# NVlabs/intrinsic3d

Measured on NVIDIA H100. Metric: gauss_newton_iterations_per_sec, higher is better.
Workload: dtype f32

## Files before the change

### intrinsic3d_b200/csrc/i3d_engine.cu

```cuda
#include <cuda_runtime.h>
#include <dlfcn.h>

#include <algorithm>
#include <chrono>
#include <climits>
#include <cmath>
#include <cstdarg>
#include <cstdio>
#include <cstdlib>
#include <cstring>
#include <string>
#include <vector>

#include "../../include/i3d_c_api.h"
#include "i3d_kernels.cuh"
#include "i3d_lighting.cuh"
#include "i3d_recolor.cuh"
#include "i3d_gridops.cuh"
#include "i3d_host.h"
#include "i3d_frames.h"
#include "i3d_fusion.h"
#include "i3d_mesh.h"
#include "i3d_render.h"
#include "i3d_texture.h"
// ... 69 lines not shown
    Dev<int32_t> up_xyz, up_vals; Dev<uint8_t> up_rgb; Dev<unsigned long long> up_keys; Dev<int> up_dup; Dev<double> up_sh;
    uint64_t hash_cap = 0;
    Dev<int32_t> sp_x, sp_y, sp_z; Dev<double> sp_sdf0, sp_sdf, sp_alb; Dev<float> sp_w; Dev<uchar4> sp_rgb;
    Dev<int32_t> act, scan_counts, scan_total;
    int n_active = 0, K = 0, stride = 0;
    Dev<float> Rt;
    Dev<FramePose> pose_ctx, pose_ctx_c;
    Dev<int32_t> obs_frame, row_frame;
    Dev<float> obs_w;
    Dev<float4> Jt;
    Dev<float2> Jtail;
    Dev<double> row_res, row_wraw;
    Dev<float> ea_w;
    Dev<double> lap;
    Dev<float> cam_acc;
    Dev<double> minv, type_w;
    Dev<int> fail_flag;
    Dev<float> v_bg, v_cg, v_s, v_jtj, v_b, v_x, v_r, v_z, v_p, v_ps, v_qg, v_tr, v_delta;
    Dev<double> v_bgd, v_cgd, v_qgd, cam_accd;
    Dev<CgCtl> ctl;
    Dev<double> red_partials, red_out;
    Dev<unsigned int> red_counters;
    size_t max_blocks = 0;
    bool keep_raw = false;
    Dev<float> dbg_v;
    I3DParams last_params{};
    bool have_iter = false;
    Timing timing;
    int64_t launches = 0;
    int64_t host_syncs = 0;
    Dev<IterDev> iter_dev;
    int last_cg_iterations = 4, prev_cg_iterations = 4;
    bool pcg_fused = true;
    int64_t step_n = -1;
    unsigned step_grid = 0; int step_K = 0; size_t step_smem = 0;
    Dev<uint8_t> color;
    bool have_color = false;
    Dev<unsigned long long> recolor_counts;
    Dev<int32_t> sv_table, sv_index, sv_nbr;
    Dev<int> sv_scalars, sv_deg;
    Dev<double> sv_acc, sv_work;
    Dev<I3DLightingInfo> sv_info;
    Dev<uint8_t> sh_has;
    int sv_S = 0;
    double* sv_x = nullptr;
    SubvolGrid sv_grid{};
    FusionState fusion;
    ScoreScratch scores;
    RgbdStore rgbd;
    SensorStore sensor;
    MeshState mesh;
    TextureState tex;
    DistanceState dist;
    RenderState render;
    TrackScratch track;
    int64_t shard_begin = 0, shard_end = -1;
    int rank = 0, world = 1;
    NcclApi::Comm comm = nullptr;
    bool shard_ready = false;
    Dev<uint8_t> held;
    Dev<uint8_t> held_mask;
    Dev<int32_t> slist;
    int64_t n_shared = 0;
    int64_t hv0 = 0, hv1 = 0;
    int64_t loc_begin = 0, loc_end = 0;
    Dev<double> xbuf;
// ... 264 lines not shown
        return;
    }
    NK(g_nccl.AllReduce(dev, dev, static_cast<size_t>(count), NCCL_FLOAT64, NCCL_SUM, e->comm, e->stream));
    if (kind >= 0) pdl_launch(e, k_epilogue, 1, 32, 0, e->ctl.p, dev, kind, respect_done);
}

void exchange(I3DEngine* e, float* v0, float* v1, float* extra_f, int n_extra_f, double* extra_d, int n_extra_d, int respect_done, int epilogue_kind = -1)
{
    if (e->world <= 1) return;
    const ShareView shv = e->share_view();
    const size_t nv = v1 ? 2 : 1;
    const size_t total = nv * static_cast<size_t>(e->n_shared) + n_extra_f + n_extra_d;
    const size_t threads = static_cast<size_t>(e->n_shared) + n_extra_f + n_extra_d;
    if (e->p2p_ready && total <= e->mbox_cap)
    {
        const unsigned int seq = ++e->xseq;
        double* buf = reinterpret_cast<double*>(e->mbox.p + I3DEngine::kMboxFlagBytes) + static_cast<size_t>(seq & 1u) * e->mbox_cap;
        pdl_launch(e, k_pack, blocks_for(threads), kThreads, 0, shv, v0, v1, extra_f, n_extra_f, extra_d, n_extra_d, buf, e->ctl.p, respect_done);
        pdl_launch(e, k_xchg_pull, blocks_for(threads), kThreads, 0, e->p2p_view(), seq, shv, v0, v1, extra_f, n_extra_f, extra_d, n_extra_d, e->ctl.p, respect_done, epilogue_kind);
        return;
    }
    e->xbuf.ensure(2 * static_cast<size_t>(e->n_shared) + CamAccLayout{e->F}.size() + 64);
    pdl_launch(e, k_pack, blocks_for(threads), kThreads, 0, shv, v0, v1, extra_f, n_extra_f, extra_d, n_extra_d, e->xbuf.p, e->ctl.p, respect_done);
    NK(g_nccl.AllReduce(e->xbuf.p, e->xbuf.p, total, NCCL_FLOAT64, NCCL_SUM, e->comm, e->stream));
    pdl_launch(e, k_unpack, blocks_for(threads), kThreads, 0, shv, v0, v1, extra_f, n_extra_f, extra_d, n_extra_d, e->xbuf.p, e->ctl.p, respect_done);
    if (epilogue_kind >= 0) pdl_launch(e, k_epilogue, 1, 32, 0, e->ctl.p, extra_d, epilogue_kind, respect_done);
}

size_t apply_smem_bytes(int F, int K)
{
    return static_cast<size_t>((6 * F + 9 + 15) & ~15) * sizeof(double) + static_cast<size_t>(14 + 6 * K) * kThreads * sizeof(float);
}

size_t accum_smem_bytes(int F, int K)
{
    return static_cast<size_t>((CamAccLayout{F}.size() + 15) & ~15) * sizeof(double) + static_cast<size_t>(K) * 8 * kThreads * sizeof(float);
}

int check_frame_limit(I3DEngine* e, int F, int K)
{
    int optin = 0;
    CK(cudaDeviceGetAttribute(&optin, cudaDevAttrMaxSharedMemoryPerBlockOptin, e->device));
    cudaFuncAttributes fa_acc{}, fa_app{};
    CK(cudaFuncGetAttributes(&fa_acc, k_eg_accum));
    CK(cudaFuncGetAttributes(&fa_app, k_eg_apply));
    const size_t lim = static_cast<size_t>(optin);
    auto fits = [&](int f) { return fa_acc.sharedSizeBytes + accum_smem_bytes(f, K) <= lim && fa_app.sharedSizeBytes + apply_smem_bytes(f, K) <= lim; };
    if (fits(F)) return 0;
    int fmax = 0;
    while (fits(fmax + 1)) ++fmax;
    return fail(e, "i3d_gn_iteration: %d frames at K = %d observations need %zu bytes of shared memory per block in k_eg_accum (device limit %d): "
                   "at most %d frames at K = %d", F, K, fa_acc.sharedSizeBytes + accum_smem_bytes(F, K), optin, fmax, K);
}

void launch_eg_apply(I3DEngine* e, const GridView& g, const RegView& rv, const EgRows& rows, const SolveVecs& sv)
{
    if (rows.n_active == 0) return;
    Timer kt(e->timing, e->stream, "k_eg_apply");
    pdl_launch(e, k_eg_apply, blocks_for(rows.n_active), kThreads, apply_smem_bytes(e->F, rows.K), g, rows, rv, sv, sv.ps, e->ctl.p, e->site(SITE_EG_APPLY));
}

void launch_operator(I3DEngine* e, const GridView& g, const RegView& rv, const EgRows& rows, const SolveVecs& sv, const Shard& sh, const float* vin,
                     float dmin, float dmax, int is_cg_iteration)
{
    launch_eg_apply(e, g, rv, rows, sv);
    {
        Timer kt(e->timing, e->stream, "k_op_partial", 1);
        pdl_launch(e, k_op_partial, blocks_for(static_cast<size_t>((e->held_count() + 3) / 4)), kThreads, 0,
            g, rv, sv, sh, e->held_count(), vin, sv.ps, e->type_w.p, dmin, dmax, e->ctl.p, e->site(SITE_OP_POST), e->site(SITE_EG_APPLY).out, is_cg_iteration);
    }
    if (e->world > 1)
    {
        Timer kt(e->timing, e->stream, "exchange", 1);
        exchange(e, sv.qg, nullptr, sv.qg + 2 * e->n, 6 * e->F + 9, e->site(SITE_OP_POST).out, 1, 1, is_cg_iteration ? EPI_OPERATOR_CG : -1);
    }
}

bool plan_cg_step(I3DEngine* e)
{
    if (e->step_n == e->n) return e->step_grid > 0;
    e->step_n = e->n; e->step_grid = 0;
    int sms = 0, optin = 0;
    CK(cudaDeviceGetAttribute(&sms, cudaDevAttrMultiProcessorCount, e->device));
    CK(cudaDeviceGetAttribute(&optin, cudaDevAttrMaxSharedMemoryPerBlockOptin, e->device));
    cudaFuncAttributes fa0{}, fa1{};
// ... 100 lines not shown
        const size_t smem = 12 * static_cast<size_t>(F) * sizeof(float);
        auto kern = (K <= 5) ? k_select_obs<5> : k_select_obs<I3D_MAX_OBS>;
        if (smem > 48 * 1024) CK(cudaFuncSetAttribute(kern, cudaFuncAttributeMaxDynamicSharedMemorySize, static_cast<int>(smem)));
        Timer kt(e->timing, e->stream, "k_select_obs");
        static const bool want_stats = std::getenv("I3D_CULL_STATS") != nullptr;
        e->cull_stats.ensure(2);
        if (want_stats) CK(cudaMemsetAsync(e->cull_stats.p, 0, 2 * sizeof(unsigned long long), st));
        const CullView cull = cull_view(e, want_stats ? e->cull_stats.p : nullptr);
        pdl_launch(e, kern, blocks_for(static_cast<size_t>(n_active)), kThreads, smem, g, e->frame_view(), e->Rt.p, sc, cull, n_active, stride, e->act.p, K,
                                                                                e->obs_frame.p, e->obs_w.p);
        if (want_stats)
        {
            unsigned long long hs[2] = {0, 0};
            CK(cudaMemcpyAsync(hs, e->cull_stats.p, sizeof(hs), cudaMemcpyDeviceToHost, st));
            CK(cudaStreamSynchronize(st));
            fprintf(stderr, "[i3d] frame culling: %llu of %llu (warp, frame) pairs visited (%.1f %%)\n", hs[0], hs[1], hs[1] ? 100.0 * hs[0] / hs[1] : 0.0);
        }
    }
    t_sel.stop();

    Timer t_build(e->timing, e->stream, "build");
    e->Jt.ensure(EgRows::kTiles * S + 1); e->Jtail.ensure(S + 1);
    e->row_frame.ensure(S + 1); e->row_res.ensure(S + 1); e->row_wraw.ensure(S + 1);
    e->ea_w.ensure(3 * static_cast<size_t>(n)); e->lap.ensure(n);
    CK(cudaFuncSetAttribute(k_eg_apply, cudaFuncAttributeMaxDynamicSharedMemorySize, static_cast<int>(apply_smem_bytes(F, K))));
    const EgRows rows = eg_rows(e);
    CamView cv{e->cam, e->pose_ctx.p, F};
    if (n_active > 0)
    {
        {
            Timer kt(e->timing, e->stream, "k_eg_build");
            launch_eg_rows<ROWS_BUILD>(e, g, cv, rows, e->obs_frame.p, e->obs_w.p);
        }
        const size_t smem = accum_smem_bytes(F, K);
        if (smem > 48 * 1024) CK(cudaFuncSetAttribute(k_eg_accum, cudaFuncAttributeMaxDynamicSharedMemorySize, static_cast<int>(smem)));
        {
            Timer kt(e->timing, e->stream, "k_eg_accum", 1);
            pdl_launch(e, k_eg_accum, blocks_for(static_cast<size_t>(n_active)), kThreads, smem, g, rows, F, e->v_bgd.p, e->v_cgd.p, e->cam_accd.p, e->site(SITE_BUILD));
        }
        pdl_launch(e, k_acc_to_float, blocks_for(std::max(U, static_cast<size_t>(lay.size()))), kThreads, 0, static_cast<int64_t>(U), lay.size(),
                   e->v_bgd.p, e->v_cgd.p, e->cam_accd.p, e->v_bg.p, e->v_cg.p, e->cam_acc.p);
    }
    const RegView rv = reg_view(e, P);
    pdl_launch(e, k_reg_build, blocks_for(static_cast<size_t>((sh.loc_end - sh.loc_begin + 3) / 4)), kThreads, 0, g, rv, sh, e->site(SITE_REG));
    {
        const double na = static_cast<double>(n_active);
        CK(cudaMemcpyAsync(e->site(SITE_BUILD).out + 3, &na, sizeof(double), cudaMemcpyHostToDevice, st));
    }
    if (multi) exchange(e, e->v_bg.p, e->v_cg.p, e->cam_acc.p, lay.size(), e->red_out.p, 2 * kSiteVals, 0);
    pdl_launch(e, k_type_weights, 1, 32, 0, e->iter_dev.p, e->site(SITE_BUILD).out, e->site(SITE_REG).out, P, n, e->type_w.p);
    if (S > 0) pdl_launch(e, k_row_weights, blocks_for(S), kThreads, 0, rows, e->type_w.p);
    SolveVecs sv = solve_vecs(e);
    pdl_launch(e, k_finish_problem, blocks_for(static_cast<size_t>((hc + 3) / 4)), kThreads, 0, g, rv, sv, sh, hc, e->type_w.p, e->cam_acc.p, P.fix_poses, P.fix_intrinsics,
                                                                              P.fix_distortion, P.gradient_tolerance, e->site(SITE_FINISH), e->cam);
    allreduce_scalars(e, e->site(SITE_FINISH).out, 3, -1, 0);
    pdl_launch(e, k_iter_finish, 1, 32, 0, e->iter_dev.p, e->site(SITE_FINISH).out, P);
    t_build.stop();
    e->have_iter = true;
    if (P.build_only)
    {
        IterDev hb{};
        CK(cudaMemcpyAsync(&hb, e->iter_dev.p, sizeof(hb), cudaMemcpyDeviceToHost, st));
        sync();
        CK(cudaGetLastError());
        info = hb.info;
        t_total.stop();
        return 0;
    }

    Timer t_solve(e->timing, e->stream, "solve");
    const float dmin = static_cast<float>(P.min_lm_diagonal), dmax = static_cast<float>(std::min(P.max_lm_diagonal, 3.0e38));
// ... 234 lines not shown

extern "C" {

int i3d_abi_version(void) { return I3D_ABI_VERSION; }
uint64_t i3d_sizeof_params(void) { return sizeof(I3DParams); }
uint64_t i3d_sizeof_iter_info(void) { return sizeof(I3DIterInfo); }

void i3d_default_params(I3DParams* p)
{
    std::memset(p, 0, sizeof(*p));
    p->lambda[0] = 0.2; p->lambda[1] = 80.0; p->lambda[2] = 120.0; p->lambda[3] = 0.1;
    p->use_er = p->use_es = p->use_ea = 1;
    p->occlusion_distance = 0.02f; p->num_observations = 5; p->lm_steps = 50;
    p->initial_trust_region_radius = 1e4; p->max_trust_region_radius = 1e16; p->min_trust_region_radius = 1e-32;
    p->min_relative_decrease = 1e-3; p->min_lm_diagonal = 1e-6; p->max_lm_diagonal = 1e32; p->eta = 0.1;
    p->function_tolerance = 1e-6; p->gradient_tolerance = 1e-10; p->parameter_tolerance = 1e-8;
    p->max_linear_solver_iterations = 500; p->min_linear_solver_iterations = 0; p->residual_reset_period = 10;
    p->max_consecutive_invalid_steps = 5;
}

int i3d_engine_create(int device, I3DEngine** out)
{
    *out = nullptr;
    int count = 0;
    cudaError_t err = cudaGetDeviceCount(&count);
    if (err != cudaSuccess || count <= 0) return fail(nullptr, "i3d_engine_create: no CUDA device available (%s); this engine has no CPU fallback", cudaGetErrorString(err));
    if (device < 0 || device >= count) return fail(nullptr, "i3d_engine_create: device %d out of range (%d devices)", device, count);
    cudaDeviceProp prop;
    if (cudaGetDeviceProperties(&prop, device) != cudaSuccess) return fail(nullptr, "i3d_engine_create: cannot query device %d", device);
    if (prop.major != 9 || prop.minor != 0) return fail(nullptr, "i3d_engine_create: device %d is sm_%d%d; this library is built for sm_90a (H100) only", device, prop.major, prop.minor);
    I3DEngine* e = new I3DEngine();
    e->device = device;
    { const char* v = std::getenv("I3D_PCG_FUSED"); e->pcg_fused = !(v && v[0] == '0'); }
    const int rc = guarded(e, [&]() {
        CK(cudaStreamCreateWithFlags(&e->stream, cudaStreamNonBlocking));
        e->timing.pool.resize(4096);
        for (auto& ev : e->timing.pool) CK(cudaEventCreate(&ev));
        return 0;
    });
    if (rc != 0) { g_create_error = e->error; delete e; return rc; }
    *out = e;
    return 0;
}

void i3d_engine_destroy(I3DEngine* e)
{
    if (!e) return;
    cudaSetDevice(e->device);
    cudaStreamSynchronize(e->stream);
    for (size_t r = 0; r < e->peer_base.size(); ++r)
        if (static_cast<int>(r) != e->rank && e->peer_base[r]) cudaIpcCloseMemHandle(e->peer_base[r]);
    if (e->comm && g_nccl.CommDestroy) g_nccl.CommDestroy(e->comm);
    for (auto& ev : e->timing.pool) cudaEventDestroy(ev);
    if (e->mesh.ev_ready) for (auto& ev : e->mesh.ev) cudaEventDestroy(ev);
    if (e->tex.ev_ready) for (auto& ev : e->tex.ev) cudaEventDestroy(ev);
    cudaStreamDestroy(e->stream);
    delete e;
}

const char* i3d_last_error(const I3DEngine* e) { return e ? e->error.c_str() : g_create_error.c_str(); }

int i3d_upload_grid(I3DEngine* e, int64_t n, const int32_t* xyz, const double* sdf0, const double* sdf_refined, const double* albedo,
                    const float* weight, const uint8_t* rgb, float voxel_size)
{
    if (!e) return 1;
    if (n <= 0 || n > (1ll << 30)) return fail(e, "i3d_upload_grid: bad voxel count %lld", static_cast<long long>(n));
// ... 1529 lines not shown
```

### intrinsic3d_b200/csrc/i3d_kernels.cuh

```cuda
#pragma once
#include <cuda_runtime.h>
#include <cooperative_groups.h>
#include <stdint.h>
#include <limits.h>
#include "i3d_math.cuh"
#include "i3d_grid.cuh"
#include "i3d_observe.cuh"
#include "../../include/i3d_types.h"

namespace i3d
{

enum : uint8_t { FL_VALID = 1, FL_ACTIVE = 2, FL_RING = 4, FL_FREE_SDF = 8, FL_FREE_ALB = 16, FL_ES_JAC = 32, FL_ROW = 64  };

struct Shard
{
    int64_t own_begin, own_end;
    int64_t hv0, hv1;
    int cam_owner;
    int defer;
    int64_t loc_begin, loc_end;
    __device__ __forceinline__ bool owns_voxel(int64_t v) const { return v >= own_begin && v < own_end; }
    __device__ __forceinline__ bool owns_unknown(int64_t j, int64_t n) const
    {
// ... 422 lines not shown
struct EgRows
{
    int n_active, K;
    int stride;
    const int32_t* act;
    float4* Jt;
    float2* Jtail;
    int32_t* row_frame;
    double* row_res;
    double* row_wraw;
    static constexpr int kTiles = 7;
    __host__ __device__ size_t slots() const { return static_cast<size_t>(K) * stride; }
    __device__ __forceinline__ void store_row(size_t slot, const float row[29]) const
    {
        const size_t S = slots();
#pragma unroll
        for (int c = 0; c < kTiles; ++c) Jt[c * S + slot] = make_float4(row[4 * c], row[4 * c + 1], row[4 * c + 2], row[4 * c + 3]);
        Jtail[slot].x = row[28];
    }
    template <bool STREAM>
    __device__ __forceinline__ float load_row(size_t slot, float jr[29]) const
    {
        const size_t S = slots();
#pragma unroll
        for (int c = 0; c < kTiles; ++c)
        {
            const float4 t = STREAM ? __ldcs(Jt + c * S + slot) : Jt[c * S + slot];
            jr[4 * c] = t.x; jr[4 * c + 1] = t.y; jr[4 * c + 2] = t.z; jr[4 * c + 3] = t.w;
        }
        const float2 t = STREAM ? __ldcs(Jtail + slot) : Jtail[slot];
        jr[28] = t.x;
        return t.y;
    }
};

__device__ __forceinline__ void make_cam_params(const CamView& cv, double pyr_scale, int W, int H, CamParams<double>* c)
{
    const double* intr = cv.cam + 6 * cv.F;
    const double* dist = intr + 4;
    c->fx = intr[0] * pyr_scale; c->fy = intr[1] * pyr_scale; c->cx = intr[2] * pyr_scale; c->cy = intr[3] * pyr_scale;
    c->k1 = dist[0]; c->k2 = dist[1]; c->k3 = dist[2]; c->p1 = dist[3]; c->p2 = dist[4];
    c->pyr_scale = pyr_scale; c->w = W; c->h = H;
}

__device__ __forceinline__ bool gather_stencil(const GridView& g, const double* __restrict__ sdf, const double* __restrict__ alb, int64_t v,
                                               int32_t idx[14], double s10[10], double a4[4])
{
    const int64_t n = g.n;
    const int32_t xp = g.nbr[NB_XP * n + v], yp = g.nbr[NB_YP * n + v], zp = g.nbr[NB_ZP * n + v];
    const int32_t x2 = g.nbr[NB_X2 * n + v], y2 = g.nbr[NB_Y2 * n + v], z2 = g.nbr[NB_Z2 * n + v];
    const int32_t xy = g.nbr[NB_XY * n + v], xz = g.nbr[NB_XZ * n + v], yz = g.nbr[NB_YZ * n + v];
    idx[0] = static_cast<int32_t>(v); idx[1] = yp; idx[2] = y2; idx[3] = yz; idx[4] = zp; idx[5] = z2; idx[6] = xp; idx[7] = xy; idx[8] = xz; idx[9] = x2;
    idx[10] = static_cast<int32_t>(v); idx[11] = xp; idx[12] = yp; idx[13] = zp;
    bool ok = true;
#pragma unroll
    for (int k = 0; k < 10; ++k) ok = ok && (idx[k] >= 0);
    if (!ok) return false;
#pragma unroll
    for (int k = 0; k < 10; ++k) s10[k] = sdf[idx[k]];
#pragma unroll
    for (int k = 0; k < 4; ++k) a4[k] = alb[idx[10 + k]];
    return true;
}

__device__ __forceinline__ double sdf_to_weight(double sdf, double truncation)
{
    const double a = fmin(fabs(sdf), truncation) / truncation;
    return fmin(fmax(1.0 - a, 0.01), 1.0);
}

struct CamAccLayout
{
    int F;
    __host__ __device__ int pose_stride() const { return 33; }
    __host__ __device__ int tail() const { return 33 * F; }
    __host__ __device__ int size() const { return 33 * F + 43; }
};

enum { ROWS_BUILD = 0, ROWS_COST = 1 };
constexpr int kRowThreads = 128;

__device__ __forceinline__ uint32_t smem_u32(const void* p) { return static_cast<uint32_t>(__cvta_generic_to_shared(p)); }
__device__ __forceinline__ void mbar_init(uint64_t* bar, uint32_t count)
{
    asm volatile("mbarrier.init.shared::cta.b64 [%0], %1;" ::"r"(smem_u32(bar)), "r"(count) : "memory");
    asm volatile("fence.mbarrier_init.release.cluster;" ::: "memory");
}
__device__ __forceinline__ void mbar_expect_tx(uint64_t* bar, uint32_t bytes)
{
    asm volatile("mbarrier.arrive.expect_tx.shared::cta.b64 _, [%0], %1;" ::"r"(smem_u32(bar)), "r"(bytes) : "memory");
}
__device__ __forceinline__ void bulk_copy_g2s(void* dst_smem, const void* src_gmem, uint32_t bytes , uint64_t* bar)
{
    asm volatile("cp.async.bulk.shared::cluster.global.mbarrier::complete_tx::bytes [%0], [%1], %2, [%3];"
                 ::"r"(smem_u32(dst_smem)), "l"(src_gmem), "r"(bytes), "r"(smem_u32(bar)) : "memory");
}
__device__ __forceinline__ void mbar_wait(uint64_t* bar, uint32_t parity)
{
    uint32_t done = 0;
    while (!done)
        asm volatile("{\n\t.reg .pred P1;\n\tmbarrier.try_wait.parity.shared::cta.b64 P1, [%1], %2;\n\tselp.b32 %0, 1, 0, P1;\n\t}"
                     : "=r"(done) : "r"(smem_u32(bar)), "r"(parity) : "memory");
}

static_assert(kVoxelGeomWords == 15, "VoxelGeom size changed: update the pose-table staging boundary and its test");
__host__ __device__ inline size_t rows_pose_bytes(int F) { return (static_cast<size_t>(F) * sizeof(FramePose) + 127) & ~static_cast<size_t>(127); }
__host__ __device__ inline size_t rows_smem_bytes(int mode, int threads, bool stage, int F)
{
    return (stage ? 128 + rows_pose_bytes(F) : 0) + static_cast<size_t>(threads) * (kVoxelGeomWords * sizeof(double) + (mode == ROWS_BUILD ? kVoxelDerivWords * sizeof(float) : 0));
// ... 68 lines not shown
                asm volatile("prefetch.global.L1 [%0];" ::"l"(pf + 128));
            }
            int32_t rf = -1; double res = 0.0, wraw = 0.0;
            if (f >= 0)
            {
                const FramePose& fp = STAGE ? s_pose[f] : cv.fpose[f];
                PointSave sv[4];
                float e[4];
                res = eg_frame_primal<MODE == ROWS_BUILD>(vg, fp, cam, LinearImage{fr.lum + img_stride * f}, sv, e);
                if (MODE == ROWS_BUILD)
                {
                    if (res != 0.0)
                    {
                        CamParams<float> cf;
                        cf.fx = static_cast<float>(cam.fx); cf.fy = static_cast<float>(cam.fy); cf.cx = static_cast<float>(cam.cx); cf.cy = static_cast<float>(cam.cy);
                        cf.k1 = static_cast<float>(cam.k1); cf.k2 = static_cast<float>(cam.k2); cf.k3 = static_cast<float>(cam.k3);
                        cf.p1 = static_cast<float>(cam.p1); cf.p2 = static_cast<float>(cam.p2);
                        cf.pyr_scale = static_cast<float>(cam.pyr_scale); cf.w = cam.w; cf.h = cam.h;
                        float row[29];
                        eg_frame_deriv(vd, fp, cf, sv, e, row);
                        rf = f;
                        wraw = static_cast<double>(obs_w[slot]) * wsdf;
                        rows.store_row(slot, row);
                    }
                }
                else acc[0] += rows.row_wraw[slot] * res * res;
            }
            if (MODE == ROWS_BUILD) { rows.row_frame[slot] = rf; rows.row_res[slot] = res; rows.row_wraw[slot] = wraw; }
        }
    }
    if (MODE == ROWS_COST) grid_reduce<1>(acc, site);
}

__global__ void __launch_bounds__(kThreads)
k_eg_accum(GridView g, EgRows rows, int F, double* __restrict__ bg, double* __restrict__ cg, double* __restrict__ cam_acc ,
           ReduceSite site )
{
    pdl_prologue();
    extern __shared__ double s_dyn_d[];
    const CamAccLayout lay{F};
    double* s_cam = s_dyn_d;
    float* s_park = reinterpret_cast<float*>(s_dyn_d + ((lay.size() + 15) & ~15));
    for (int i = threadIdx.x; i < lay.size(); i += blockDim.x) s_cam[i] = 0.0;
    __syncthreads();
    const int tid = threadIdx.x, lane = tid & 31;
    const int a = blockIdx.x * blockDim.x + tid;
    const bool in_range = a < rows.n_active;
    double acc[3] = {0.0, 0.0, 0.0};
    float gsum[14], csum[14];
#pragma unroll
    for (int m = 0; m < 14; ++m) { gsum[m] = 0.0f; csum[m] = 0.0f; }
    float tl[64];
#pragma unroll
    for (int i = 0; i < 64; ++i) tl[i] = 0.0f;
    int fk[I3D_MAX_OBS];
#pragma unroll
    for (int k = 0; k < I3D_MAX_OBS; ++k)
    {
        fk[k] = -1;
        if (k >= rows.K) continue;
        const size_t slot = static_cast<size_t>(k) * rows.stride + (in_range ? a : 0);
        const int f = in_range ? rows.row_frame[slot] : -1;
        fk[k] = f;
        if (f >= 0)
        {
            float row[29];
            rows.load_row<false>(slot, row);
            const double wraw = rows.row_wraw[slot], res = rows.row_res[slot];
            const float wf = static_cast<float>(wraw), wr = static_cast<float>(wraw * res);
            acc[0] += wraw; acc[1] += wraw * res * res; acc[2] += 1.0;
#pragma unroll
            for (int m = 0; m < 14; ++m) { gsum[m] += wr * row[m]; csum[m] += wf * row[m] * row[m]; }
#pragma unroll
            for (int m = 0; m < 9; ++m) { tl[m] += wr * row[20 + m]; tl[9 + m] += wf * row[20 + m] * row[20 + m]; }
            int t = 18;
#pragma unroll
            for (int r = 0; r < 4; ++r)
#pragma unroll
                for (int c = r; c < 4; ++c) tl[t++] += wf * row[20 + r] * row[20 + c];
#pragma unroll
            for (int r = 0; r < 5; ++r)
#pragma unroll
                for (int c = r; c < 5; ++c) tl[t++] += wf * row[24 + r] * row[24 + c];
#pragma unroll
            for (int c = 0; c < 6; ++c) s_park[(k * 8 + c) * kThreads + tid] = row[14 + c];
            s_park[(k * 8 + 6) * kThreads + tid] = wf;
            s_park[(k * 8 + 7) * kThreads + tid] = wr;
        }
    }
    if (__ballot_sync(0xffffffffu, acc[2] > 0.0) != 0u)
    {
        warp_reduce_scatter<64>(tl, lane);
#pragma unroll
        for (int i = 0; i < 2; ++i)
        {
            const int id = rs_index<64>(i, lane);
            if (id < 43 && tl[i] != 0.0f) atomicAdd(s_cam + lay.tail() + id, static_cast<double>(tl[i]));
        }
    }
    unsigned todo = 0u;
#pragma unroll
    for (int k = 0; k < I3D_MAX_OBS; ++k) if (fk[k] >= 0) todo |= 1u << k;
    while (true)
    {
        const unsigned pending = __ballot_sync(0xffffffffu, todo != 0u);
        if (pending == 0u) break;
        const int leader = __ffs(pending) - 1;
        const int mine_f = (todo != 0u) ? fk_select(fk, __ffs(todo) - 1) : -1;
        const int f0 = __shfl_sync(0xffffffffu, mine_f, leader);
        float jp[6] = {0.0f, 0.0f, 0.0f, 0.0f, 0.0f, 0.0f};
        float wf = 0.0f, wr = 0.0f;
#pragma unroll
        for (int k = 0; k < I3D_MAX_OBS; ++k)
        {
            if (k >= rows.K) break;
            if (((todo >> k) & 1u) && fk[k] == f0)
            {
#pragma unroll
                for (int c = 0; c < 6; ++c) jp[c] = s_park[(k * 8 + c) * kThreads + tid];
                wf = s_park[(k * 8 + 6) * kThreads + tid];
                wr = s_park[(k * 8 + 7) * kThreads + tid];
                todo &= ~(1u << k);
            }
        }
        float v[32];
#pragma unroll
        for (int c = 0; c < 6; ++c) { v[c] = wr * jp[c]; v[6 + c] = wf * jp[c] * jp[c]; }
        int t = 12;
        float last = 0.0f;
#pragma unroll
        for (int r = 0; r < 6; ++r)
#pragma unroll
            for (int c = r; c < 6; ++c)
            {
                const float pr = wf * jp[r] * jp[c];
                if (t < 32) v[t] = pr; else last = pr;
                ++t;
            }
        warp_reduce_scatter<32>(v, lane);
#pragma unroll
        for (int o = 16; o > 0; o >>= 1) last += __shfl_xor_sync(0xffffffffu, last, o);
        double* dst = s_cam + lay.pose_stride() * f0;
        if (v[0] != 0.0f) atomicAdd(dst + lane, static_cast<double>(v[0]));
        if (lane == 0 && last != 0.0f) atomicAdd(dst + 32, static_cast<double>(last));
    }
    if (in_range && acc[2] > 0.0)
    {
        const int64_t v = rows.act[a];
        const int64_t n = g.n;
        const int32_t xp = g.nbr[NB_XP * n + v], yp = g.nbr[NB_YP * n + v], zp = g.nbr[NB_ZP * n + v];
        int64_t idx[14];
        idx[0] = v; idx[1] = yp; idx[2] = g.nbr[NB_Y2 * n + v]; idx[3] = g.nbr[NB_YZ * n + v]; idx[4] = zp; idx[5] = g.nbr[NB_Z2 * n + v];
        idx[6] = xp; idx[7] = g.nbr[NB_XY * n + v]; idx[8] = g.nbr[NB_XZ * n + v]; idx[9] = g.nbr[NB_X2 * n + v];
        idx[10] = n + v; idx[11] = n + xp; idx[12] = n + yp; idx[13] = n + zp;
#pragma unroll
        for (int m = 0; m < 14; ++m)
            if (csum[m] != 0.0f) { atomicAdd(bg + idx[m], static_cast<double>(gsum[m])); atomicAdd(cg + idx[m], static_cast<double>(csum[m])); }
    }
    __syncthreads();
    for (int i = threadIdx.x; i < lay.size(); i += blockDim.x) { const float vv = static_cast<float>(s_cam[i]); if (vv != 0.0f) atomicAdd(cam_acc + i, static_cast<double>(vv)); }
    grid_reduce<3>(acc, site);
}

__global__ void k_acc_to_float(int64_t U, int ncam, const double* __restrict__ bgd, const double* __restrict__ cgd, const double* __restrict__ camd,
                               float* __restrict__ bg, float* __restrict__ cg, float* __restrict__ cam_acc)
{
    pdl_prologue();
    const int64_t j = blockIdx.x * static_cast<int64_t>(blockDim.x) + threadIdx.x;
    if (j < U) { bg[j] = static_cast<float>(bgd[j]); cg[j] = static_cast<float>(cgd[j]); }
    if (j < ncam) cam_acc[j] = static_cast<float>(camd[j]);
}

__global__ void k_row_weights(EgRows rows, const double* __restrict__ type_w)
{
    pdl_prologue();
    const size_t s = blockIdx.x * static_cast<size_t>(blockDim.x) + threadIdx.x;
    if (s >= rows.slots()) return;
    rows.Jtail[s].y = static_cast<float>(rows.row_wraw[s] * type_w[0]);
}

struct RegView
{
    const uint8_t* flags;
    float* ea_w;
    double* lap;
    int use_er, use_es, use_ea;
};

__device__ __forceinline__ bool albedo_pair_weight(uchar4 ca, uchar4 cb, float* w)
{
    const float la = intensity_u8(ca), lb = intensity_u8(cb);
    const float k = 1.0f / 255.0f;
    const float d0 = FS(FD(FM(static_cast<float>(ca.x), k), la), FD(FM(static_cast<float>(cb.x), k), lb));
    const float d1 = FS(FD(FM(static_cast<float>(ca.y), k), la), FD(FM(static_cast<float>(cb.y), k), lb));
// ... 1394 lines not shown
```

Before: 140.3.

## Compact per-block frame table in eg_accum to cut shared memory and registers

k_eg_accum no longer keeps a shared-memory accumulator for every camera frame. It records which frames a block touches in a bitmask, prefix-scans that mask into a compact slot table, and accumulates pose blocks in chunks of at most C slots (default 64), flushing each chunk to global. The kernel is also split into phases so the large register arrays (gsum/csum, then tl) are not live at the same time, adds launch bounds of 3 blocks per SM, and uses streaming loads for the Jacobian tiles. The aim is lower shared memory and register use per block so more blocks stay resident. The cost is extra syncs, the bitmask scan, and multiple passes when a block touches more than C frames.

Result: no change. 141.1 (median of 6 runs) (+0.6%).

```diff
diff --git a/intrinsic3d_b200/csrc/i3d_engine.cu b/intrinsic3d_b200/csrc/i3d_engine.cu
--- a/intrinsic3d_b200/csrc/i3d_engine.cu
+++ b/intrinsic3d_b200/csrc/i3d_engine.cu
@@ -125,6 +125,7 @@
     Dev<IterDev> iter_dev;
     int last_cg_iterations = 4, prev_cg_iterations = 4;
     bool pcg_fused = true;
+    int accum_slots = kAccumSlots;
     int64_t step_n = -1;
     unsigned step_grid = 0; int step_K = 0; size_t step_smem = 0;
     Dev<uint8_t> color;
@@ -455,10 +456,13 @@
     return static_cast<size_t>((6 * F + 9 + 15) & ~15) * sizeof(double) + static_cast<size_t>(14 + 6 * K) * kThreads * sizeof(float);
 }
 
-size_t accum_smem_bytes(int F, int K)
+size_t frame_limit_smem_bytes(int F, int K)
 {
     return static_cast<size_t>((CamAccLayout{F}.size() + 15) & ~15) * sizeof(double) + static_cast<size_t>(K) * 8 * kThreads * sizeof(float);
 }
+
+int accum_slots(const I3DEngine* e, int F) { return std::min(e->accum_slots, F); }
+size_t accum_smem_bytes(const I3DEngine* e, int F, int K) { return AccumSmem{F, K, accum_slots(e, F)}.bytes(); }
 
 int check_frame_limit(I3DEngine* e, int F, int K)
 {
@@ -468,12 +472,14 @@
     CK(cudaFuncGetAttributes(&fa_acc, k_eg_accum));
     CK(cudaFuncGetAttributes(&fa_app, k_eg_apply));
     const size_t lim = static_cast<size_t>(optin);
-    auto fits = [&](int f) { return fa_acc.sharedSizeBytes + accum_smem_bytes(f, K) <= lim && fa_app.sharedSizeBytes + apply_smem_bytes(f, K) <= lim; };
+    auto fits = [&](int f) {
+        return fa_acc.sharedSizeBytes + std::max(frame_limit_smem_bytes(f, K), accum_smem_bytes(e, f, K)) <= lim && fa_app.sharedSizeBytes + apply_smem_bytes(f, K) <= lim;
+    };
     if (fits(F)) return 0;
     int fmax = 0;
     while (fits(fmax + 1)) ++fmax;
     return fail(e, "i3d_gn_iteration: %d frames at K = %d observations need %zu bytes of shared memory per block in k_eg_accum (device limit %d): "
-                   "at most %d frames at K = %d", F, K, fa_acc.sharedSizeBytes + accum_smem_bytes(F, K), optin, fmax, K);
+                   "at most %d frames at K = %d", F, K, fa_acc.sharedSizeBytes + std::max(frame_limit_smem_bytes(F, K), accum_smem_bytes(e, F, K)), optin, fmax, K);
 }
 
 void launch_eg_apply(I3DEngine* e, const GridView& g, const RegView& rv, const EgRows& rows, const SolveVecs& sv)
@@ -640,11 +646,11 @@
             Timer kt(e->timing, e->stream, "k_eg_build");
             launch_eg_rows<ROWS_BUILD>(e, g, cv, rows, e->obs_frame.p, e->obs_w.p);
         }
-        const size_t smem = accum_smem_bytes(F, K);
-        if (smem > 48 * 1024) CK(cudaFuncSetAttribute(k_eg_accum, cudaFuncAttributeMaxDynamicSharedMemorySize, static_cast<int>(smem)));
+        const size_t smem = accum_smem_bytes(e, F, K);
+        CK(cudaFuncSetAttribute(k_eg_accum, cudaFuncAttributeMaxDynamicSharedMemorySize, static_cast<int>(smem)));
         {
             Timer kt(e->timing, e->stream, "k_eg_accum", 1);
-            pdl_launch(e, k_eg_accum, blocks_for(static_cast<size_t>(n_active)), kThreads, smem, g, rows, F, e->v_bgd.p, e->v_cgd.p, e->cam_accd.p, e->site(SITE_BUILD));
+            pdl_launch(e, k_eg_accum, blocks_for(static_cast<size_t>(n_active)), kThreads, smem, g, rows, F, accum_slots(e, F), e->v_bgd.p, e->v_cgd.p, e->cam_accd.p, e->site(SITE_BUILD));
         }
         pdl_launch(e, k_acc_to_float, blocks_for(std::max(U, static_cast<size_t>(lay.size()))), kThreads, 0, static_cast<int64_t>(U), lay.size(),
                    e->v_bgd.p, e->v_cgd.p, e->cam_accd.p, e->v_bg.p, e->v_cg.p, e->cam_acc.p);
@@ -945,6 +951,7 @@
     I3DEngine* e = new I3DEngine();
     e->device = device;
     { const char* v = std::getenv("I3D_PCG_FUSED"); e->pcg_fused = !(v && v[0] == '0'); }
+    { const char* v = std::getenv("I3D_ACCUM_SLOTS"); if (v && std::atoi(v) >= 1) e->accum_slots = std::atoi(v); }
     const int rc = guarded(e, [&]() {
         CK(cudaStreamCreateWithFlags(&e->stream, cudaStreamNonBlocking));
         e->timing.pool.resize(4096);
diff --git a/intrinsic3d_b200/csrc/i3d_kernels.cuh b/intrinsic3d_b200/csrc/i3d_kernels.cuh
--- a/intrinsic3d_b200/csrc/i3d_kernels.cuh
+++ b/intrinsic3d_b200/csrc/i3d_kernels.cuh
@@ -478,6 +478,19 @@
         jr[28] = t.x;
         return t.y;
     }
+    template <int C0, int C1, bool STREAM>
+    __device__ __forceinline__ void load_tiles(size_t slot, float* jr) const
+    {
+        const size_t S = slots();
+#pragma unroll
+        for (int c = C0; c < C1; ++c)
+        {
+            const float4 t = STREAM ? __ldcs(Jt + c * S + slot) : Jt[c * S + slot];
+            jr[4 * (c - C0)] = t.x; jr[4 * (c - C0) + 1] = t.y; jr[4 * (c - C0) + 2] = t.z; jr[4 * (c - C0) + 3] = t.w;
+        }
+    }
+    template <bool STREAM>
+    __device__ __forceinline__ float load_col28(size_t slot) const { return STREAM ? __ldcs(Jtail + slot).x : Jtail[slot].x; }
 };
 
 __device__ __forceinline__ void make_cam_params(const CamView& cv, double pyr_scale, int W, int H, CamParams<double>* c)
@@ -521,6 +534,20 @@
     __host__ __device__ int pose_stride() const { return 33; }
     __host__ __device__ int tail() const { return 33 * F; }
     __host__ __device__ int size() const { return 33 * F + 43; }
+};
+
+constexpr int kAccumSlots = 64;
+
+struct AccumSmem
+{
+    int F, K, C;
+    __host__ __device__ int table() const { return (CamAccLayout{C}.size() + 15) & ~15; }
+    __host__ __device__ int words() const { return (F + 31) / 32; }
+    __host__ __device__ size_t bytes() const
+    {
+        return static_cast<size_t>(table()) * sizeof(double) + static_cast<size_t>(K) * 8 * kThreads * sizeof(float) +
+               static_cast<size_t>(2 * words() + F) * sizeof(int);
+    }
 };
 
 enum { ROWS_BUILD = 0, ROWS_COST = 1 };
@@ -655,134 +682,202 @@
     if (MODE == ROWS_COST) grid_reduce<1>(acc, site);
 }
 
-__global__ void __launch_bounds__(kThreads)
-k_eg_accum(GridView g, EgRows rows, int F, double* __restrict__ bg, double* __restrict__ cg, double* __restrict__ cam_acc ,
+__global__ void __launch_bounds__(kThreads, 3)
+k_eg_accum(GridView g, EgRows rows, int F, int C, double* __restrict__ bg, double* __restrict__ cg, double* __restrict__ cam_acc ,
            ReduceSite site )
 {
     pdl_prologue();
     extern __shared__ double s_dyn_d[];
-    const CamAccLayout lay{F};
+    const AccumSmem sm{F, rows.K, C};
+    const CamAccLayout lay{F}, tab{C};
     double* s_cam = s_dyn_d;
-    float* s_park = reinterpret_cast<float*>(s_dyn_d + ((lay.size() + 15) & ~15));
-    for (int i = threadIdx.x; i < lay.size(); i += blockDim.x) s_cam[i] = 0.0;
+    float* s_park = reinterpret_cast<float*>(s_dyn_d + sm.table());
+    unsigned* s_bits = reinterpret_cast<unsigned*>(s_park + rows.K * 8 * kThreads);
+    int* s_first = reinterpret_cast<int*>(s_bits + sm.words());
+    int* s_frame = s_first + sm.words();
+    __shared__ int s_nframes;
+    for (int i = threadIdx.x; i < tab.size(); i += blockDim.x) s_cam[i] = 0.0;
+    for (int i = threadIdx.x; i < sm.words(); i += blockDim.x) s_bits[i] = 0u;
     __syncthreads();
     const int tid = threadIdx.x, lane = tid & 31;
     const int a = blockIdx.x * blockDim.x + tid;
     const bool in_range = a < rows.n_active;
     double acc[3] = {0.0, 0.0, 0.0};
-    float gsum[14], csum[14];
-#pragma unroll
-    for (int m = 0; m < 14; ++m) { gsum[m] = 0.0f; csum[m] = 0.0f; }
-    float tl[64];
-#pragma unroll
-    for (int i = 0; i < 64; ++i) tl[i] = 0.0f;
-    int fk[I3D_MAX_OBS];
+    unsigned rmask = 0u;
+    {
+        float gsum[14], csum[14];
+#pragma unroll
+        for (int m = 0; m < 14; ++m) { gsum[m] = 0.0f; csum[m] = 0.0f; }
+#pragma unroll
+        for (int k = 0; k < I3D_MAX_OBS; ++k)
+        {
+            if (k >= rows.K) continue;
+            const size_t slot = static_cast<size_t>(k) * rows.stride + (in_range ? a : 0);
+            const int f = in_range ? rows.row_frame[slot] : -1;
+            if (f >= 0)
+            {
+                rmask |= 1u << k;
+                atomicOr(s_bits + (f >> 5), 1u << (f & 31));
+                float row[20];
+                rows.load_tiles<0, 5, true>(slot, row);
+                const double wraw = __ldcs(rows.row_wraw + slot), res = __ldcs(rows.row_res + slot);
+                const float wf = static_cast<float>(wraw), wr = static_cast<float>(wraw * res);
+                acc[0] += wraw; acc[1] += wraw * res * res; acc[2] += 1.0;
+#pragma unroll
+                for (int m = 0; m < 14; ++m) { gsum[m] += wr * row[m]; csum[m] += wf * row[m] * row[m]; }
+#pragma unroll
+                for (int c = 0; c < 6; ++c) s_park[(k * 8 + c) * kThreads + tid] = row[14 + c];
+                s_park[(k * 8 + 6) * kThreads + tid] = wf;
+                s_park[(k * 8 + 7) * kThreads + tid] = wr;
+            }
+        }
+        if (in_range && acc[2] > 0.0)
+        {
+            const int64_t v = rows.act[a];
+            const int64_t n = g.n;
+            const int32_t xp = g.nbr[NB_XP * n + v], yp = g.nbr[NB_YP * n + v], zp = g.nbr[NB_ZP * n + v];
+            int64_t idx[14];
+            idx[0] = v; idx[1] = yp; idx[2] = g.nbr[NB_Y2 * n + v]; idx[3] = g.nbr[NB_YZ * n + v]; idx[4] = zp; idx[5] = g.nbr[NB_Z2 * n + v];
+            idx[6] = xp; idx[7] = g.nbr[NB_XY * n + v]; idx[8] = g.nbr[NB_XZ * n + v]; idx[9] = g.nbr[NB_X2 * n + v];
+            idx[10] = n + v; idx[11] = n + xp; idx[12] = n + yp; idx[13] = n + zp;
+#pragma unroll
+            for (int m = 0; m < 14; ++m)
+                if (csum[m] != 0.0f) { atomicAdd(bg + idx[m], static_cast<double>(gsum[m])); atomicAdd(cg + idx[m], static_cast<double>(csum[m])); }
+        }
+    }
+    grid_reduce<3>(acc, site);
+    __syncthreads();
+    if (tid < 32)
+    {
+        int base = 0;
+        for (int j0 = 0; j0 < sm.words(); j0 += 32)
+        {
+            const int j = j0 + lane;
+            const unsigned bits = (j < sm.words()) ? s_bits[j] : 0u;
+            const int cnt = __popc(bits);
+            int incl = cnt;
+#pragma unroll
+            for (int o = 1; o < 32; o <<= 1)
+            {
+                const int t = __shfl_up_sync(0xffffffffu, incl, o);
+                if (lane >= o) incl += t;
+            }
+            int s = base + incl - cnt;
+            if (j < sm.words()) s_first[j] = s;
+            for (unsigned m = bits; m != 0u; m &= m - 1u) s_frame[s++] = 32 * j + __ffs(m) - 1;
+            base += __shfl_sync(0xffffffffu, incl, 31);
+        }
+        if (lane == 0) s_nframes = base;
+    }
+    {
+        float tl[64];
+#pragma unroll
+        for (int i = 0; i < 64; ++i) tl[i] = 0.0f;
+#pragma unroll
+        for (int k = 0; k < I3D_MAX_OBS; ++k)
+        {
+            if (!((rmask >> k) & 1u)) continue;
+            const size_t slot = static_cast<size_t>(k) * rows.stride + a;
+            float row[9];
+            rows.load_tiles<5, 7, true>(slot, row);
+            row[8] = rows.load_col28<true>(slot);
+            const float wf = s_park[(k * 8 + 6) * kThreads + tid], wr = s_park[(k * 8 + 7) * kThreads + tid];
+#pragma unroll
+            for (int c = 0; c < 9; ++c) { tl[c] += wr * row[c]; tl[9 + c] += wf * row[c] * row[c]; }
+            int t = 18;
+#pragma unroll
+            for (int r = 0; r < 4; ++r)
+#pragma unroll
+                for (int c = r; c < 4; ++c) tl[t++] += wf * row[r] * row[c];
+#pragma unroll
+            for (int r = 0; r < 5; ++r)
+#pragma unroll
+                for (int c = r; c < 5; ++c) tl[t++] += wf * row[4 + r] * row[4 + c];
+        }
+        if (__ballot_sync(0xffffffffu, rmask != 0u) != 0u)
+        {
+            warp_reduce_scatter<64>(tl, lane);
+#pragma unroll
+            for (int i = 0; i < 2; ++i)
+            {
+                const int id = rs_index<64>(i, lane);
+                if (id < 43 && tl[i] != 0.0f) atomicAdd(s_cam + tab.tail() + id, static_cast<double>(tl[i]));
+            }
+        }
+    }
+    __syncthreads();
+    for (int i = tid; i < 43; i += blockDim.x) { const float vv = static_cast<float>(s_cam[tab.tail() + i]); if (vv != 0.0f) atomicAdd(cam_acc + lay.tail() + i, static_cast<double>(vv)); }
+    int sk[I3D_MAX_OBS];
 #pragma unroll
     for (int k = 0; k < I3D_MAX_OBS; ++k)
     {
-        fk[k] = -1;
-        if (k >= rows.K) continue;
-        const size_t slot = static_cast<size_t>(k) * rows.stride + (in_range ? a : 0);
-        const int f = in_range ? rows.row_frame[slot] : -1;
-        fk[k] = f;
-        if (f >= 0)
-        {
-            float row[29];
-            rows.load_row<false>(slot, row);
-            const double wraw = rows.row_wraw[slot], res = rows.row_res[slot];
-            const float wf = static_cast<float>(wraw), wr = static_cast<float>(wraw * res);
-            acc[0] += wraw; acc[1] += wraw * res * res; acc[2] += 1.0;
-#pragma unroll
-            for (int m = 0; m < 14; ++m) { gsum[m] += wr * row[m]; csum[m] += wf * row[m] * row[m]; }
-#pragma unroll
-            for (int m = 0; m < 9; ++m) { tl[m] += wr * row[20 + m]; tl[9 + m] += wf * row[20 + m] * row[20 + m]; }
-            int t = 18;
-#pragma unroll
-            for (int r = 0; r < 4; ++r)
-#pragma unroll
-                for (int c = r; c < 4; ++c) tl[t++] += wf * row[20 + r] * row[20 + c];
-#pragma unroll
-            for (int r = 0; r < 5; ++r)
-#pragma unroll
-                for (int c = r; c < 5; ++c) tl[t++] += wf * row[24 + r] * row[24 + c];
-#pragma unroll
-            for (int c = 0; c < 6; ++c) s_park[(k * 8 + c) * kThreads + tid] = row[14 + c];
-            s_park[(k * 8 + 6) * kThreads + tid] = wf;
-            s_park[(k * 8 + 7) * kThreads + tid] = wr;
-        }
-    }
-    if (__ballot_sync(0xffffffffu, acc[2] > 0.0) != 0u)
-    {
-        warp_reduce_scatter<64>(tl, lane);
-#pragma unroll
-        for (int i = 0; i < 2; ++i)
-        {
-            const int id = rs_index<64>(i, lane);
-            if (id < 43 && tl[i] != 0.0f) atomicAdd(s_cam + lay.tail() + id, static_cast<double>(tl[i]));
-        }
-    }
-    unsigned todo = 0u;
-#pragma unroll
-    for (int k = 0; k < I3D_MAX_OBS; ++k) if (fk[k] >= 0) todo |= 1u << k;
-    while (true)
-    {
-        const unsigned pending = __ballot_sync(0xffffffffu, todo != 0u);
-        if (pending == 0u) break;
-        const int leader = __ffs(pending) - 1;
-        const int mine_f = (todo != 0u) ? fk_select(fk, __ffs(todo) - 1) : -1;
-        const int f0 = __shfl_sync(0xffffffffu, mine_f, leader);
-        float jp[6] = {0.0f, 0.0f, 0.0f, 0.0f, 0.0f, 0.0f};
-        float wf = 0.0f, wr = 0.0f;
-#pragma unroll
-        for (int k = 0; k < I3D_MAX_OBS; ++k)
-        {
-            if (k >= rows.K) break;
-            if (((todo >> k) & 1u) && fk[k] == f0)
+        const int f = ((rmask >> k) & 1u) ? rows.row_frame[static_cast<size_t>(k) * rows.stride + a] : -1;
+        sk[k] = (f >= 0) ? s_first[f >> 5] + __popc(s_bits[f >> 5] & ((1u << (f & 31)) - 1u)) : -1;
+    }
+    const int nframes = s_nframes;
+    for (int first = 0; first < nframes; first += C)
+    {
+        if (first > 0)
+        {
+            __syncthreads();
+            for (int i = tid; i < 33 * C; i += blockDim.x) s_cam[i] = 0.0;
+            __syncthreads();
+        }
+        unsigned todo = 0u;
+#pragma unroll
+        for (int k = 0; k < I3D_MAX_OBS; ++k) if (sk[k] >= first && sk[k] < first + C) todo |= 1u << k;
+        while (true)
+        {
+            const unsigned pending = __ballot_sync(0xffffffffu, todo != 0u);
+            if (pending == 0u) break;
+            const int leader = __ffs(pending) - 1;
+            const int mine_s = (todo != 0u) ? fk_select(sk, __ffs(todo) - 1) : -1;
+            const int s0 = __shfl_sync(0xffffffffu, mine_s, leader);
+            float jp[6] = {0.0f, 0.0f, 0.0f, 0.0f, 0.0f, 0.0f};
+            float wf = 0.0f, wr = 0.0f;
+#pragma unroll
+            for (int k = 0; k < I3D_MAX_OBS; ++k)
             {
-#pragma unroll
-                for (int c = 0; c < 6; ++c) jp[c] = s_park[(k * 8 + c) * kThreads + tid];
-                wf = s_park[(k * 8 + 6) * kThreads + tid];
-                wr = s_park[(k * 8 + 7) * kThreads + tid];
-                todo &= ~(1u << k);
+                if (k >= rows.K) break;
+                if (((todo >> k) & 1u) && sk[k] == s0)
+                {
+#pragma unroll
+                    for (int c = 0; c < 6; ++c) jp[c] = s_park[(k * 8 + c) * kThreads + tid];
+                    wf = s_park[(k * 8 + 6) * kThreads + tid];
+                    wr = s_park[(k * 8 + 7) * kThreads + tid];
+                    todo &= ~(1u << k);
+                }
             }
-        }
-        float v[32];
-#pragma unroll
-        for (int c = 0; c < 6; ++c) { v[c] = wr * jp[c]; v[6 + c] = wf * jp[c] * jp[c]; }
-        int t = 12;
-        float last = 0.0f;
-#pragma unroll
-        for (int r = 0; r < 6; ++r)
-#pragma unroll
-            for (int c = r; c < 6; ++c)
-            {
-                const float pr = wf * jp[r] * jp[c];
-                if (t < 32) v[t] = pr; else last = pr;
-                ++t;
-            }
-        warp_reduce_scatter<32>(v, lane);
-#pragma unroll
-        for (int o = 16; o > 0; o >>= 1) last += __shfl_xor_sync(0xffffffffu, last, o);
-        double* dst = s_cam + lay.pose_stride() * f0;
-        if (v[0] != 0.0f) atomicAdd(dst + lane, static_cast<double>(v[0]));
-        if (lane == 0 && last != 0.0f) atomicAdd(dst + 32, static_cast<double>(last));
-    }
-    if (in_range && acc[2] > 0.0)
-    {
-        const int64_t v = rows.act[a];
-        const int64_t n = g.n;
-        const int32_t xp = g.nbr[NB_XP * n + v], yp = g.nbr[NB_YP * n + v], zp = g.nbr[NB_ZP * n + v];
-        int64_t idx[14];
-        idx[0] = v; idx[1] = yp; idx[2] = g.nbr[NB_Y2 * n + v]; idx[3] = g.nbr[NB_YZ * n + v]; idx[4] = zp; idx[5] = g.nbr[NB_Z2 * n + v];
-        idx[6] = xp; idx[7] = g.nbr[NB_XY * n + v]; idx[8] = g.nbr[NB_XZ * n + v]; idx[9] = g.nbr[NB_X2 * n + v];
-        idx[10] = n + v; idx[11] = n + xp; idx[12] = n + yp; idx[13] = n + zp;
-#pragma unroll
-        for (int m = 0; m < 14; ++m)
-            if (csum[m] != 0.0f) { atomicAdd(bg + idx[m], static_cast<double>(gsum[m])); atomicAdd(cg + idx[m], static_cast<double>(csum[m])); }
-    }
-    __syncthreads();
-    for (int i = threadIdx.x; i < lay.size(); i += blockDim.x) { const float vv = static_cast<float>(s_cam[i]); if (vv != 0.0f) atomicAdd(cam_acc + i, static_cast<double>(vv)); }
-    grid_reduce<3>(acc, site);
+            float v[32];
+#pragma unroll
+            for (int c = 0; c < 6; ++c) { v[c] = wr * jp[c]; v[6 + c] = wf * jp[c] * jp[c]; }
+            int t = 12;
+            float last = 0.0f;
+#pragma unroll
+            for (int r = 0; r < 6; ++r)
+#pragma unroll
+                for (int c = r; c < 6; ++c)
+                {
+                    const float pr = wf * jp[r] * jp[c];
+                    if (t < 32) v[t] = pr; else last = pr;
+                    ++t;
+                }
+            warp_reduce_scatter<32>(v, lane);
+#pragma unroll
+            for (int o = 16; o > 0; o >>= 1) last += __shfl_xor_sync(0xffffffffu, last, o);
+            double* dst = s_cam + tab.pose_stride() * (s0 - first);
+            if (v[0] != 0.0f) atomicAdd(dst + lane, static_cast<double>(v[0]));
+            if (lane == 0 && last != 0.0f) atomicAdd(dst + 32, static_cast<double>(last));
+        }
+        __syncthreads();
+        const int nent = 33 * min(C, nframes - first);
+        for (int i = tid; i < nent; i += blockDim.x)
+        {
+            const float vv = static_cast<float>(s_cam[i]);
+            const int s = i / 33;
+            if (vv != 0.0f) atomicAdd(cam_acc + lay.pose_stride() * s_frame[first + s] + (i - 33 * s), static_cast<double>(vv));
+        }
+    }
 }
 
 __global__ void k_acc_to_float(int64_t U, int ncam, const double* __restrict__ bgd, const double* __restrict__ cgd, const double* __restrict__ camd,
```
